# skokec/DAU-ConvNet

Hardware: AMD Instinct MI355X
Metric: DAU fwd+bwd GSamples/s (N*H*W/s) (higher is better)
Workload: dtype f32

## Files before the change

### dau-convnet_amd/csrc/k_dense_split.hip

```cpp
#include <algorithm>
#include <cstdint>
#include <cstdlib>
#include <type_traits>

#include "dau_tiled.hpp"

#ifndef DAU_SPLIT_R
#define DAU_SPLIT_R 3
#endif
#ifndef DAU_SPLIT_NS
#define DAU_SPLIT_NS s3
#endif

namespace dau {
namespace DAU_SPLIT_NS {

typedef _Float16 f16x8 __attribute__((ext_vector_type(8)));
typedef __attribute__((ext_vector_type(16))) float f32x16;
typedef __attribute__((ext_vector_type(4))) float f32x4;
typedef __attribute__((ext_vector_type(4))) unsigned u32x4;
typedef __attribute__((address_space(3))) void* lds_ptr_t;
typedef __attribute__((address_space(1))) const void* glb_ptr_t;

namespace {

constexpr int kDR = DAU_SPLIT_R;
constexpr int kDK = 2 * kDR + 1;
constexpr int kDSpan = kDK - 1;
constexpr int kDTaps = kDK * kDK;
constexpr int kDRows = 8;
constexpr int kDFB = 128;
constexpr int kAhead = 2;
#ifndef DAU_SPLIT_FLUSH_TAPS
#define DAU_SPLIT_FLUSH_TAPS 0
#endif
constexpr int kFlushTaps = DAU_SPLIT_FLUSH_TAPS > 0 ? DAU_SPLIT_FLUSH_TAPS : kDK;
#ifndef DAU_SPLIT_FLUSH_ROWS
#define DAU_SPLIT_FLUSH_ROWS 4
#endif
constexpr int kFlushRows = DAU_SPLIT_FLUSH_ROWS;
#if !defined(DAU_SPLIT_K32)
#if !defined(DAU_SPLIT_MFMA32) && DAU_SPLIT_R == 3
#define DAU_SPLIT_K32 1
#else
#define DAU_SPLIT_K32 0
#endif
#endif
constexpr bool kK32 = DAU_SPLIT_K32 != 0;

inline size_t round_up(size_t v, size_t a) { return (v + a - 1) / a * a; }

struct SplitScales {
    unsigned max_w_bits;
    float sw, inv_sw;
    float pad[5];
};
__host__ __device__ __forceinline__ const float* scales_sx(const SplitScales* sc) { return reinterpret_cast<const float*>(sc + 1); }
__host__ __device__ __forceinline__ const float* scales_inv_sx(const SplitScales* sc, int N) { return reinterpret_cast<const float*>(sc + 1) + N; }
constexpr int kPartials = 1024;
inline int absmax_groups_per_image(int N, long per) {
    const long fit = std::max(1, kPartials / N), want = (per / 4 + 255) / 256 + 1;
    return (int)std::min(fit, want);
}
inline size_t scales_bytes(int N) { return sizeof(SplitScales) + (size_t)2 * N * sizeof(float); }

constexpr int kMaxSub = 4;
struct SplitGeom {
    int sub;
    int nsub_a, nb_a, nsub_b, nb_b;
    int nrb8, nrb4;
    int tall;
    int Hs, Ws, nchunk, CoutP;
    size_t hdr_bytes, xs_bytes, ws_bytes;
};

SplitGeom split_geometry(const DenseConfig& c) {
    SplitGeom g{};
    g.sub = (c.W + 7) / 8;
    const int nblocks = (g.sub + kMaxSub - 1) / kMaxSub, base = g.sub / nblocks, rem = g.sub % nblocks;
    if (rem) { g.nsub_a = base + 1; g.nb_a = rem; g.nsub_b = base; g.nb_b = nblocks - rem; }
    else { g.nsub_a = base; g.nb_a = nblocks; g.nsub_b = 0; g.nb_b = 0; }
    const int left = c.H % kDRows;
    const long wgs = (long)c.N * ((c.H + kDRows - 1) / kDRows) * nblocks * ((c.Cout + kDFB - 1) / kDFB);
    const int rows4 = DAU_TUNE_INT("DAU_SPLIT_ROWS4", 1);
    g.nrb4 = (left >= 1 && left <= 4 && rows4 != 0 && (wgs >= 1024 || rows4 == 2)) ? 1 : 0;
    g.nrb8 = c.H / kDRows + (left && !g.nrb4 ? 1 : 0);
    g.Hs = g.nrb8 * kDRows + g.nrb4 * 4 + kDSpan;
    {
        const int t4 = (c.W + 3) / 4;
        const long rows8 = (long)g.nrb8 * kDRows;
        const long flat = (long)(g.nrb4 ? rows8 + 4 : (c.H + 3) / 4 * 4) * g.sub * 8;
        const long tall = rows8 * t4 * 4 + (g.nrb4 ? 4L * g.sub * 8 : 0);
        const int want = DAU_TUNE_INT("DAU_SPLIT_TALL", 1);
        g.tall = (want != 0 && g.nrb8 > 0 && (t4 == 5 || t4 == 7) && (tall * 20 <= flat * 19 || want == 2)) ? t4 : 0;
    }
    g.Ws = g.sub * 8 + kDSpan;
    g.nchunk = (c.Cin + 15) / 16;
    g.CoutP = (int)round_up(c.Cout, kDFB);
    g.hdr_bytes = round_up(scales_bytes(c.N) + (size_t)2 * (kPartials + c.N) * sizeof(unsigned), 256);
    g.xs_bytes = round_up((size_t)c.N * g.nchunk * 4 * g.Hs * g.Ws * 16 + 4096, 256);
    g.ws_bytes = round_up(((size_t)g.nchunk * kDTaps + 8) * 2 * g.CoutP * 32, 256);
    return g;
}

constexpr int lds_pitch(int nsub) {
    int p = nsub * 8 + kDSpan;
    while (p % 16 != 8) ++p;
    return p;
}
constexpr int lds_pitch_narrow(int ntiles) {
    int p = ntiles * 4 + kDSpan;
    while (p % 16 != 4 && p % 16 != 12) ++p;
    return p;
}

}

__device__ __forceinline__ unsigned finite_bits(unsigned b) { return b < 0x7f800000u ? b : 0u; }

__device__ __forceinline__ long absmax_head(const void* p, long per, int elem_bytes, int vec_bytes) {
    const uintptr_t a = reinterpret_cast<uintptr_t>(p);
    if (a % elem_bytes) return per;
    const long head = (long)((vec_bytes - a % vec_bytes) % vec_bytes) / elem_bytes;
    return head < per ? head : per;
}

__global__ void __launch_bounds__(256) split_absmax_kernel(const float* __restrict__ in, long per, int gpi, int act, const UnitRef* __restrict__ table,
                                                           long units, unsigned* __restrict__ partial, int cap, const Guard guard) {
    if (!guard_pass(guard)) return;
    unsigned mx = 0, mw = 0;
    const int n = blockIdx.x / gpi, j = blockIdx.x - n * gpi;
    const long stride = (long)gpi * blockDim.x, t0 = j * (long)blockDim.x + threadIdx.x;
    if (act == kActF16) {
        auto wide = [](unsigned h) { return finite_bits(__float_as_uint(f16_bits_to_float(h)) & 0x7fffffffu); };
        const unsigned short* e = reinterpret_cast<const unsigned short*>(in) + n * per;
        const long head = absmax_head(e, per, 2, 8), n4 = (per - head) / 4;
        const uint2* p = reinterpret_cast<const uint2*>(e + head);
        for (long i = t0; i < n4; i += stride) {
            const uint2 v = p[i];
            mx = max(mx, max(max(wide(v.x & 0xffffu), wide(v.x >> 16)), max(wide(v.y & 0xffffu), wide(v.y >> 16))));
        }
        for (long i = t0; i < per - n4 * 4; i += stride) mx = max(mx, wide(e[i < head ? i : i + n4 * 4]));
    } else if (act == kActBF16) {
        const unsigned short* e = reinterpret_cast<const unsigned short*>(in) + n * per;
        const long head = absmax_head(e, per, 2, 8), n4 = (per - head) / 4;
        const uint2* p = reinterpret_cast<const uint2*>(e + head);
        for (long i = t0; i < n4; i += stride) {
            const uint2 v = p[i];
            mx = max(mx, max(max(finite_bits((v.x << 16) & 0x7fffffffu), finite_bits(v.x & 0x7fff0000u)),
                             max(finite_bits((v.y << 16) & 0x7fffffffu), finite_bits(v.y & 0x7fff0000u))));
        }
        for (long i = t0; i < per - n4 * 4; i += stride) mx = max(mx, finite_bits(((unsigned)e[i < head ? i : i + n4 * 4] << 16) & 0x7fffffffu));
    } else {
        const float* e = in + n * per;
        const long head = absmax_head(e, per, 4, 16), n4 = (per - head) / 4;
        const uint4* p = reinterpret_cast<const uint4*>(e + head);
        for (long i = t0; i < n4; i += stride) {
            const uint4 v = p[i];
            mx = max(mx, max(max(finite_bits(v.x & 0x7fffffffu), finite_bits(v.y & 0x7fffffffu)),
                             max(finite_bits(v.z & 0x7fffffffu), finite_bits(v.w & 0x7fffffffu))));
        }
        for (long i = t0; i < per - n4 * 4; i += stride) mx = max(mx, finite_bits(__float_as_uint(e[i < head ? i : i + n4 * 4]) & 0x7fffffffu));
    }
    for (long u = blockIdx.x * (long)blockDim.x + threadIdx.x; u < units; u += (long)gridDim.x * blockDim.x) {
        const UnitRef r = table[u];
        mw = max(mw, finite_bits(__float_as_uint(fabsf(r.w00) + fabsf(r.w01) + fabsf(r.w10) + fabsf(r.w11))));
    }
    __shared__ unsigned sx[4], sw[4];
    for (int m = 32; m >= 1; m >>= 1) { mx = max(mx, (unsigned)__shfl_xor((int)mx, m)); mw = max(mw, (unsigned)__shfl_xor((int)mw, m)); }
    if ((threadIdx.x & 63) == 0) { sx[threadIdx.x >> 6] = mx; sw[threadIdx.x >> 6] = mw; }
    __syncthreads();
    if (threadIdx.x == 0) {
        partial[blockIdx.x] = max(max(sx[0], sx[1]), max(sx[2], sx[3]));
        partial[cap + blockIdx.x] = max(max(sw[0], sw[1]), max(sw[2], sw[3]));
    }
}

__device__ __forceinline__ float limb_scale(float m) {
    if (!(m > 0.0f) || !(m < INFINITY)) return 1.0f;
    int e = ilogbf(m);
    e = 13 - e;
    e = e > 100 ? 100 : (e < -100 ? -100 : e);
    return ldexpf(1.0f, e);
}

__global__ void __launch_bounds__(256) split_scales_kernel(const unsigned* __restrict__ partial, int N, int gpi, int cap, int G,
                                                           SplitScales* __restrict__ out, const Guard guard) {
    if (!guard_pass(guard)) return;
    const int n = blockIdx.x;
    const unsigned* src = n < N ? partial + (long)n * gpi : partial + cap;
    const int cnt = n < N ? gpi : N * gpi;
    unsigned m = 0;
    for (int i = threadIdx.x; i < cnt; i += 256) m = max(m, src[i]);
    __shared__ unsigned sm[4];
    for (int k = 32; k >= 1; k >>= 1) m = max(m, (unsigned)__shfl_xor((int)m, k));
    if ((threadIdx.x & 63) == 0) sm[threadIdx.x >> 6] = m;
    __syncthreads();
    if (threadIdx.x == 0) {
        m = max(max(sm[0], sm[1]), max(sm[2], sm[3]));
        float* sx = reinterpret_cast<float*>(out + 1);
        if (n < N) {
            const float s = limb_scale(__uint_as_float(m));
            sx[n] = s; sx[N + n] = 1.0f / s;
        } else {
            const float s = limb_scale(__uint_as_float(m) * (float)G);
            out->max_w_bits = m; out->sw = s; out->inv_sw = 1.0f / s;
        }
    }
}

constexpr int kScT = 64;
__global__ void __launch_bounds__(kScT) split_densify_kernel(const UnitRef* __restrict__ table, int Cin, int G, int Cout, int CoutP, int nchunk,
                                                             const SplitScales* __restrict__ sc, _Float16* __restrict__ wsd, const Guard guard) {
    __shared__ float acc[kDTaps * kScT];
    if (!guard_pass(guard)) return;
    constexpr int FPB = kScT / 16;
    const int tid = threadIdx.x, sl = tid & 15;
    const int fq = blockIdx.x % (CoutP / FPB), chunk = blockIdx.x / (CoutP / FPB);
    const int f = fq * FPB + (tid >> 4), c = chunk * 16 + sl;
#pragma unroll 7
    for (int tap = 0; tap < kDTaps; ++tap) acc[tap * kScT + tid] = 0.0f;
    if (c < Cin && f < Cout) {
        for (int g = 0; g < G; ++g) {
            const UnitRef u = table[((long)c * G + g) * Cout + f];
            const int ty = u.oy + kDR, tx = u.ox + kDR;
            const bool y0 = ty >= 0 && ty < kDK, y1 = ty + 1 >= 0 && ty + 1 < kDK, x0 = tx >= 0 && tx < kDK, x1 = tx + 1 >= 0 && tx + 1 < kDK;
            if (y0 && x0) acc[(ty * kDK + tx) * kScT + tid] += u.w00;
            if (y0 && x1) acc[(ty * kDK + tx + 1) * kScT + tid] += u.w01;
            if (y1 && x0) acc[((ty + 1) * kDK + tx) * kScT + tid] += u.w10;
            if (y1 && x1) acc[((ty + 1) * kDK + tx + 1) * kScT + tid] += u.w11;
        }
    }
    const float sw = sc->sw;
    _Float16* dst = wsd + ((long)chunk * kDTaps * 2 * CoutP + f) * 16 + sl;
    const long limb = (long)CoutP * 16, tapstride = 2 * limb;
#pragma unroll 7
    for (int tap = 0; tap < kDTaps; ++tap) {
        const float v = acc[tap * kScT + tid] * sw;
        const _Float16 hi = (_Float16)v;
        dst[tap * tapstride] = hi;
        dst[tap * tapstride + limb] = (_Float16)(v - (float)hi);
    }
}

constexpr int kSP = 80;
struct SplitStageArgs {
    const float* in;
    const float* taps;
    const SplitScales* sc;
    _Float16* xs;
    int N, C, H, W, mirrored;
    int Hs, Ws, nchunk;
    int RB, nbands, nsegs;
    int vec;
    Guard guard;
};

__device__ __forceinline__ int fast_div(int i, int d, float inv) {
    int q = (int)(((float)i + 0.5f) * inv);
    const int r = i - q * d;
    q += (r >= d) - (r < 0);
    return q;
}

template <int K, int NCH>
__device__ __forceinline__ void split_stage_rows(float* rawl, const float* px, int col, int ch0, int wave, int nw, int lh, int ncols) {
    constexpr int kr = (K - 1) / 2;
    if (col >= ncols) return;
    float gx[K];
#pragma unroll
    for (int j = 0; j < K; ++j) gx[j] = px[j];
    for (int r = wave; r < lh; r += nw) {
        float* row = rawl + (r * 8 + ch0) * kSP + 8 + col;
        float acc[NCH];
#pragma unroll
        for (int ch = 0; ch < NCH; ++ch) {
            acc[ch] = 0.0f;
#pragma unroll
            for (int i = 0; i < K; ++i) acc[ch] = fmaf(row[ch * kSP + i - kr], gx[i], acc[ch]);
        }
#pragma unroll
        for (int ch = 0; ch < NCH; ++ch) row[ch * kSP] = acc[ch];
    }
}

template <int K, int NCH>
__device__ __forceinline__ void split_stage_walk(const float* rawl, const float* py, float sx, int col, int ch0, int ya, int yb,
                                                 int y0, int x0, int x1, int Ws, u32x4* xhi, u32x4* xlo) {
    constexpr int kr = (K - 1) / 2;
    const int x = x0 + col;
    if (x >= x1) return;
    float gy[K];
#pragma unroll
    for (int j = 0; j < K; ++j) gy[j] = py[j];
    float ring[K][NCH];
    const int nin = yb - ya + 2 * kr;
    char* dhi = reinterpret_cast<char*>(xhi + (long)kDR * Ws + kDR + x) + ch0 * 2;
    char* dlo = reinterpret_cast<char*>(xlo + (long)kDR * Ws + kDR + x) + ch0 * 2;
    for (int s0 = 0; s0 < nin; s0 += K) {
#pragma unroll
        for (int j = 0; j < K; ++j) {
            const int s = s0 + j;
            if (s < nin) {
                const float* row = rawl + ((ya - y0 + s) * 8 + ch0) * kSP + 8 + col;
#pragma unroll
                for (int ch = 0; ch < NCH; ++ch) ring[j][ch] = row[ch * kSP];
                if (s >= K - 1) {
                    typedef _Float16 f16xn __attribute__((ext_vector_type(NCH)));
                    f16xn oh, ol;
#pragma unroll
                    for (int ch = 0; ch < NCH; ++ch) {
                        float acc = 0.0f;
#pragma unroll
                        for (int i = 0; i < K; ++i) acc = fmaf(ring[(j + 1 + i) % K][ch], gy[i], acc);
                        acc *= sx;
                        const _Float16 hi = (_Float16)acc;
                        oh[ch] = hi;
                        ol[ch] = (_Float16)(acc - (float)hi);
                    }
                    const long o = (long)(ya + s - (K - 1)) * Ws * 16;
                    *reinterpret_cast<f16xn*>(dhi + o) = oh;
                    *reinterpret_cast<f16xn*>(dlo + o) = ol;
                }
            }
        }
    }
}

#ifndef DAU_SPLIT_STAGE_THREADS
#define DAU_SPLIT_STAGE_THREADS 512
#endif
constexpr int kStageThreads = DAU_SPLIT_STAGE_THREADS;
template <int KN, int A>
__global__ void __launch_bounds__(kStageThreads) split_stage_kernel(const SplitStageArgs a) {
    constexpr int K = KN & (kNhwcArg - 1);
    constexpr bool NHWC = (KN & kNhwcArg) != 0;
    extern __shared__ __attribute__((aligned(16))) float rawl[];
    if (!guard_pass(a.guard)) return;
    constexpr int kr = (K - 1) / 2;
    constexpr int PPR = kSP / 4;
    const int lane = threadIdx.x & 63, wave = threadIdx.x >> 6, nw = blockDim.x >> 6;
    int t = blockIdx.x;
    const int seg = t % a.nsegs; t /= a.nsegs;
    const int band = t % a.nbands; t /= a.nbands;
    const int grp = t % (2 * a.nchunk);
    const int n = t / (2 * a.nchunk);
    const int y0 = band * a.RB, y1 = y0 + a.RB < a.H ? y0 + a.RB : a.H;
    const int x0 = seg * 64, x1 = x0 + 64 < a.W ? x0 + 64 : a.W;
    const int lh = y1 - y0 + 2 * kr;
    const long plane = (long)a.H * a.W;
    if constexpr (NHWC) {
        constexpr int CPP = A == kActF32 ? 4 : 8, PARTS = 8 / CPP;
        const int pieces = lh * kSP * PARTS;
        constexpr int UB = (13 * 256 + kStageThreads - 1) / kStageThreads;
        for (int i0 = threadIdx.x; i0 < pieces; i0 += kStageThreads * UB) {
            float v[UB][CPP];
#pragma unroll
            for (int u = 0; u < UB; ++u) {
                const int i = i0 + u * kStageThreads, part = i % PARTS, rj = i / PARTS, r = rj / kSP, j = rj - r * kSP;
                const int c = grp * 8 + part * CPP, y = y0 - kr + r, x = x0 - 8 + j;
                const bool pix = y >= 0 && y < a.H && x >= 0 && x < a.W && i < pieces;
                if (a.vec) {
                    const bool ok = pix && c < a.C;
                    const long idx = ok ? nhwc_index(n, c, y, x, a.C, a.H, a.W) : 0;
                    if constexpr (A == kActF32) {
                        const float4 w = *reinterpret_cast<const float4*>(a.in + idx);
                        v[u][0] = mask_act(w.x, ok); v[u][1] = mask_act(w.y, ok); v[u][2] = mask_act(w.z, ok); v[u][3] = mask_act(w.w, ok);
                    } else {
                        const uint4 w = *reinterpret_cast<const uint4*>(reinterpret_cast<const unsigned short*>(a.in) + idx);
                        const unsigned q[4] = {w.x, w.y, w.z, w.w};
#pragma unroll
                        for (int k = 0; k < 4; ++k) {
                            if constexpr (A == kActF16) {
                                v[u][2 * k] = mask_act(f16_bits_to_float(q[k] & 0xffffu), ok);
                                v[u][2 * k + 1] = mask_act(f16_bits_to_float(q[k] >> 16), ok);
                            } else {
                                const unsigned m = ok ? 0xffffffffu : 0u;
                                v[u][2 * k] = __uint_as_float((q[k] << 16) & m);
                                v[u][2 * k + 1] = __uint_as_float(q[k] & 0xffff0000u & m);
                            }
                        }
                    }
                } else {
#pragma unroll
                    for (int k = 0; k < CPP; ++k) {
                        const bool ok = pix && c + k < a.C;
                        v[u][k] = mask_act(load_act_t<A>(a.in, ok ? nhwc_index(n, c + k, y, x, a.C, a.H, a.W) : 0), ok);
                    }
                }
            }
#pragma unroll
            for (int u = 0; u < UB; ++u) {
                const int i = i0 + u * kStageThreads, part = i % PARTS, rj = i / PARTS, r = rj / kSP, j = rj - r * kSP;
                if (i < pieces) {
#pragma unroll
                    for (int k = 0; k < CPP; ++k) rawl[(r * 8 + part * CPP + k) * kSP + j] = v[u][k];
                }
            }
        }
    } else
    {
        const int pieces = lh * 8 * PPR;
        constexpr int UB = (13 * 256 + kStageThreads - 1) / kStageThreads;
        for (int i0 = threadIdx.x; i0 < pieces; i0 += kStageThreads * UB) {
            float4 v[UB];
#pragma unroll
            for (int u = 0; u < UB; ++u) {
                const int i = i0 + u * kStageThreads, rc = i / PPR, q = i - rc * PPR, r = rc >> 3, ch = rc & 7;
                const int c = grp * 8 + ch, y = y0 - kr + r, xs = x0 - 8 + 4 * q;
                const bool row_in = c < a.C && y >= 0 && y < a.H && i < pieces;
                const long base = ((long)n * a.C + (c < a.C ? c : 0)) * plane;
                if (a.vec) {
                    const bool ok = row_in && xs >= 0 && xs + 4 <= a.W;
                    const long idx = base + (ok ? (long)y * a.W + xs : 0);
                    if constexpr (A == kActF16) {
                        const uint2 w = *reinterpret_cast<const uint2*>(reinterpret_cast<const unsigned short*>(a.in) + idx);
                        v[u] = make_float4(mask_act(f16_bits_to_float(w.x & 0xffffu), ok), mask_act(f16_bits_to_float(w.x >> 16), ok),
                                           mask_act(f16_bits_to_float(w.y & 0xffffu), ok), mask_act(f16_bits_to_float(w.y >> 16), ok));
                    } else if constexpr (A == kActBF16) {
                        const uint2 w = *reinterpret_cast<const uint2*>(reinterpret_cast<const unsigned short*>(a.in) + idx);
                        const unsigned m = ok ? 0xffffffffu : 0u;
                        v[u] = make_float4(__uint_as_float((w.x << 16) & m), __uint_as_float(w.x & 0xffff0000u & m),
                                           __uint_as_float((w.y << 16) & m), __uint_as_float(w.y & 0xffff0000u & m));
                    } else {
                        const float4 w = *reinterpret_cast<const float4*>(a.in + idx);
                        v[u] = make_float4(mask_act(w.x, ok), mask_act(w.y, ok), mask_act(w.z, ok), mask_act(w.w, ok));
                    }
                } else {
                    float e[4];
#pragma unroll
                    for (int k = 0; k < 4; ++k) {
                        const bool ok = row_in && xs + k >= 0 && xs + k < a.W;
                        e[k] = mask_act(load_act_t<A>(a.in, base + (ok ? (long)y * a.W + xs + k : 0)), ok);
                    }
                    v[u] = make_float4(e[0], e[1], e[2], e[3]);
                }
            }
#pragma unroll
            for (int u = 0; u < UB; ++u) {
                const int i = i0 + u * kStageThreads;
                if (i < pieces) *reinterpret_cast<float4*>(rawl + (long)i * 4) = v[u];
            }
        }
    }
    const int chunk = grp >> 1, half = grp & 1;
    const long splane = (long)a.Hs * a.Ws;
    u32x4* xhi = reinterpret_cast<u32x4*>(a.xs) + ((((long)n * a.nchunk + chunk) * 2 + 0) * 2 + half) * splane;
    u32x4* xlo = xhi + 2 * splane;
    {
        const int rs0 = band == 0 ? 0 : y0 + kDR, rs1 = band == a.nbands - 1 ? a.Hs : y1 + kDR;
        const int cs0 = seg == 0 ? 0 : x0 + kDR, cs1 = seg == a.nsegs - 1 ? a.Ws : x1 + kDR;
        const int cw = cs1 - cs0, cnt = (rs1 - rs0) * cw;
        const float inv = 1.0f / (float)cw;
        const u32x4 z = {0u, 0u, 0u, 0u};
        for (int i = threadIdx.x; i < cnt; i += blockDim.x) {
            const int rr = fast_div(i, cw, inv), r = rs0 + rr, cc = cs0 + i - rr * cw;
            if (r >= y0 + kDR && r < y1 + kDR && cc >= x0 + kDR && cc < x1 + kDR) continue;
            xhi[(long)r * a.Ws + cc] = z;
            xlo[(long)r * a.Ws + cc] = z;
        }
    }
    __syncthreads();
    const float* px = a.taps + (a.mirrored ? kTapGXR : kTapGX) * kTapPitch;
    const float* py = a.taps + (a.mirrored ? kTapGYR : kTapGY) * kTapPitch;
    if (x1 - x0 <= 32) split_stage_rows<K, 4>(rawl, px, lane & 31, (lane >> 5) * 4, wave, nw, lh, x1 - x0);
    else split_stage_rows<K, 8>(rawl, px, lane, 0, wave, nw, lh, x1 - x0);
    __syncthreads();
    const int SR = (y1 - y0 + nw - 1) / nw;
    const int ya = y0 + wave * SR, yb = ya + SR < y1 ? ya + SR : y1;
    if (ya >= yb) return;
    const float sx = scales_sx(a.sc)[n];
    if (x1 - x0 <= 32) split_stage_walk<K, 4>(rawl, py, sx, lane & 31, (lane >> 5) * 4, ya, yb, y0, x0, x1, a.Ws, xhi, xlo);
    else split_stage_walk<K, 8>(rawl, py, sx, lane, 0, ya, yb, y0, x0, x1, a.Ws, xhi, xlo);
}

struct SplitArgs {
    const _Float16* xs;
    const _Float16* wsd;
    const SplitScales* sc;
    float* out;
    const float* partial;
    int N, Cout, CoutP, H, W, Hs, Ws, nchunk, ncb, nrb, out_act;
    int col0;
    int row0;
    Guard guard;
};
struct SplitArgsEpi : SplitArgs {
    const float* bias;
    int relu;
    const float* residual;
    int res_vec;
};

constexpr int kNhwcVecOut = 0x100;
template <int NSUBN, int RG = 2, bool TT = false, bool H16 = false, bool ADD = false>
__global__ void __launch_bounds__(512) split_gather_kernel(const typename std::conditional<(NSUBN & kEpiArg) != 0, SplitArgsEpi, SplitArgs>::type a) {
    constexpr int NSUB = NSUBN & (kNhwcArg - 1);
    constexpr bool NHWC = (NSUBN & kNhwcArg) != 0;
    constexpr bool EPI = (NSUBN & kEpiArg) != 0;
    static_assert(!TT || RG == 2, "tall tiles: blocks of eight rows");
    constexpr int TW = TT ? 4 : 8;
    constexpr int P = TT ? lds_pitch_narrow(NSUB) : lds_pitch(NSUB);
    constexpr int kRowsWG = 4 * RG;
    constexpr int NT0 = (RG == 2 && !TT) ? NSUB : (NSUB + 1) / 2;
    constexpr int NT1 = TT ? NSUB / 2 : NT0;
    constexpr int WR = kRowsWG + kDSpan;
    constexpr int PLANE = kK32 ? (WR * P + 15) / 16 * 16 : WR * P;
    constexpr int HALF = PLANE * 16;
    constexpr int BUFU = 4 * PLANE;
    constexpr int NPIECE = (BUFU + 63) / 64;
    constexpr int BUF1 = NPIECE * 1024;
    constexpr int BUF = kK32 ? 2 * BUF1 : BUF1;
    constexpr int PPW = (NPIECE + 7) / 8;
    extern __shared__ __attribute__((aligned(16))) char smem[];
    if (!guard_pass(a.guard)) return;
    const int lane = threadIdx.x & 63;
    const int wave = __builtin_amdgcn_readfirstlane(threadIdx.x >> 6);
    const int fw = wave & 3, pw = wave >> 2;
    const int prow = (RG == 2 && !TT) ? 4 * pw : 0, ptile = (RG == 2 && !TT) ? 0 : pw * NT0;
    int t;
#ifdef DAU_SPLIT_NO_XCD_MAP
    t = blockIdx.x;
#else
    {
        const int nblk = gridDim.x, xcd = blockIdx.x % 8, idx = blockIdx.x / 8;
        const int per = nblk / 8, rem = nblk % 8;
        t = (xcd < rem ? xcd * (per + 1) : rem * (per + 1) + (xcd - rem) * per) + idx;
    }
#endif
    const int fb = t % (a.CoutP / kDFB); t /= (a.CoutP / kDFB);
    const int cb = t % a.ncb; t /= a.ncb;
    const int rb = t % a.nrb;
    const int n = t / a.nrb;
    const int h = lane >> 5, nn = lane & 31;

    const long xs_plane = (long)a.Hs * a.Ws;
    const int colb = a.col0 + cb * NSUB * TW;
    const int rowb = a.row0 + rb * kRowsWG;
    const u32x4* xsrc = reinterpret_cast<const u32x4*>(a.xs) + ((long)n * a.nchunk * 4) * xs_plane + (long)rowb * a.Ws + colb;
    int goff[PPW];
#pragma unroll
    for (int i = 0; i < PPW; ++i) {
        int piece = wave + 8 * i;
        piece = piece < NPIECE ? piece : NPIECE - 1;
        int L = piece * 64 + lane;
        L = L < BUFU ? L : BUFU - 1;
        const int ph = L / PLANE;
        int rem = L - ph * PLANE;
        rem = rem < WR * P ? rem : WR * P - 1;
        const int r = rem / P, c = rem - r * P;
        goff[i] = (int)(ph * xs_plane + (long)r * a.Ws + c);
    }
    auto issue = [&](int chunk, int buf) {
        const u32x4* src = xsrc + (long)chunk * 4 * xs_plane;
#pragma unroll
        for (int i = 0; i < PPW; ++i) {
            int piece = wave + 8 * i;
            piece = piece < NPIECE ? piece : NPIECE - 1;
            __builtin_amdgcn_global_load_lds((glb_ptr_t)(src + goff[i]), (lds_ptr_t)(smem + buf * BUF + piece * 1024), 16, 0, 0);
        }
        if constexpr (kK32) {
            if (chunk + 1 < a.nchunk) {
#pragma unroll
                for (int i = 0; i < PPW; ++i) {
                    int piece = wave + 8 * i;
                    piece = piece < NPIECE ? piece : NPIECE - 1;
                    __builtin_amdgcn_global_load_lds((glb_ptr_t)(src + 4 * xs_plane + goff[i]), (lds_ptr_t)(smem + buf * BUF + BUF1 + piece * 1024), 16, 0, 0);
                }
            }
        }
    };

    const int prr = TT ? nn >> 2 : nn >> 3, pcc = TT ? nn & 3 : nn & 7;
    float* const out_ptr = a.out;
    const float* const part_ptr = a.partial;
    const bool out_bf16 = NHWC ? (a.out_act & 0xff) != 0 : a.out_act != 0;
    const bool vec_out = NHWC && (a.out_act & kNhwcVecOut) != 0;
    const int out_c = a.Cout, out_h = a.H, out_w = a.W;
    const float* bias_ptr = nullptr;
    const float* res_ptr = nullptr;
    bool relu = false, vec_res = false;
    if constexpr (EPI) { bias_ptr = a.bias; relu = a.relu != 0; }
    auto read_residual = [&](float tie) __attribute__((always_inline)) {
        if constexpr (EPI) {
            unsigned long kargs = (unsigned long)__builtin_amdgcn_kernarg_segment_ptr();
            asm volatile("" : "+s"(kargs) : "v"(tie));
            const auto* late = reinterpret_cast<const __attribute__((address_space(4))) SplitArgsEpi*>(kargs);
            res_ptr = late->residual;
            vec_res = NHWC && late->res_vec != 0;
        }
    };
    auto finished = [&](float v, int f, float r) __attribute__((always_inline)) {
        const int fc = f < out_c ? f : out_c - 1;
        return epilogue_value(v, bias_ptr ? bias_ptr[fc] : 0.0f, bias_ptr != nullptr, relu, r, res_ptr != nullptr);
    };
    auto residual_at = [&](long o) __attribute__((always_inline)) {
        if constexpr (H16) return load_act_t<kActF16>(res_ptr, o);
        else return out_bf16 ? load_act_t<kActBF16>(res_ptr, o) : res_ptr[o];
    };
    auto joined = [&](float s, float inv_w, float inv_x, float part) __attribute__((always_inline)) {
        float v = s * inv_w * inv_x + part;
        if constexpr (H16) asm("" : "+v"(v));
        return v;
    };
    auto store4 = [&](int y, int x, bool tile, int f0, const float (&s)[4], float inv_w, float inv_x) __attribute__((always_inline)) {
        const long plane = (long)out_h * out_w;
        if (!(y < out_h && x < out_w && tile)) return;
        if constexpr (NHWC) {
            const long pix = ((long)n * out_h + y) * out_w + x;
            float v[4];
            float r[4] = {0.0f, 0.0f, 0.0f, 0.0f};
            if constexpr (EPI) {
                if (res_ptr) {
                    const long o = pix * out_c + f0;
                    if (vec_res) {
                        if (f0 < out_c) {
                            if constexpr (H16) {
                                typedef _Float16 f16x4 __attribute__((ext_vector_type(4)));
                                const f16x4 q = *reinterpret_cast<const f16x4*>(reinterpret_cast<const unsigned short*>(res_ptr) + o);
#pragma unroll
                                for (int k = 0; k < 4; ++k) r[k] = (float)q[k];
                            } else if (out_bf16) {
                                const uint2 q = *reinterpret_cast<const uint2*>(reinterpret_cast<const unsigned short*>(res_ptr) + o);
                                r[0] = __uint_as_float(q.x << 16); r[1] = __uint_as_float(q.x & 0xffff0000u);
                                r[2] = __uint_as_float(q.y << 16); r[3] = __uint_as_float(q.y & 0xffff0000u);
                            } else {
// ... 230 lines not shown
            xb[0][0] = read(0, 0); xb[0][1] = read(0, 1); xb[1][0] = read(1, 0); xb[1][1] = read(1, 1);
            __builtin_amdgcn_sched_group_barrier(0x100, 4, 0);
#pragma unroll
            for (int u = 0; u < U; ++u) {
                const int tx = u / NG, p = u % NG;
                if (u + 2 < U) { xb[(u + 2) % 3][0] = read(u + 2, 0); xb[(u + 2) % 3][1] = read(u + 2, 1); }
                const f16x8 xh = xb[u % 3][0], xl = xb[u % 3][1];
                const f16x8 h0 = ah[tx][0], h1 = ah[tx][1], l0 = al[tx][0], l1 = al[tx][1];
                const bool fresh = kFlushRows == 1 && tx % kFlushTaps == 0;
                acc[p][0] = __builtin_amdgcn_mfma_f32_16x16x32_f16(h0, xh, fresh ? zero : acc[p][0], 0, 0, 0);
                acc[p][1] = __builtin_amdgcn_mfma_f32_16x16x32_f16(h1, xh, fresh ? zero : acc[p][1], 0, 0, 0);
                if (p == 0) {
                    if (tx + kAhead < kDK) {
#pragma unroll
                        for (int m = 0; m < 2; ++m) { ah[tx + kAhead][m] = load_a(wcur, (tx + kAhead) * wtap, m); al[tx + kAhead][m] = load_a(wcur, (tx + kAhead) * wtap + wlo, m); }
                    }
                    if (tx == kDK - 3 || tx == kDK - 2) {
                        const int i = tx - (kDK - 3);
#pragma unroll
                        for (int m = 0; m < 2; ++m) { an[i][m] = load_a(wnxt, i * wtap, m); bn[i][m] = load_a(wnxt, i * wtap + wlo, m); }
                    }
                }
                acc[p][0] = __builtin_amdgcn_mfma_f32_16x16x32_f16(l0, xh, acc[p][0], 0, 0, 0);
                acc[p][1] = __builtin_amdgcn_mfma_f32_16x16x32_f16(l1, xh, acc[p][1], 0, 0, 0);
                acc[p][0] = __builtin_amdgcn_mfma_f32_16x16x32_f16(h0, xl, acc[p][0], 0, 0, 0);
                acc[p][1] = __builtin_amdgcn_mfma_f32_16x16x32_f16(h1, xl, acc[p][1], 0, 0, 0);
                if (u + 2 < U) __builtin_amdgcn_sched_group_barrier(0x100, 2, 0);
                __builtin_amdgcn_sched_group_barrier(0x008, 2, 0);
                if (p == 0 && tx + kAhead < kDK && tx == kDK - 3) __builtin_amdgcn_sched_group_barrier(0x020, 8, 0);
                else if (p == 0 && (tx + kAhead < kDK || tx == kDK - 2)) __builtin_amdgcn_sched_group_barrier(0x020, 4, 0);
                __builtin_amdgcn_sched_group_barrier(0x008, 4, 0);
                if ((tx + 1) % kFlushTaps == 0 && tx + 1 < kDK) { sum[p][0] += acc[p][0]; sum[p][1] += acc[p][1]; }
            }
#pragma unroll
            for (int m = 0; m < 2; ++m) { ah[0][m] = an[0][m]; al[0][m] = bn[0][m]; ah[1][m] = an[1][m]; al[1][m] = bn[1][m]; }
            if constexpr (kFlushRows == 1) {
#pragma unroll
                for (int p = 0; p < NG; ++p) { sum[p][0] += acc[p][0]; sum[p][1] += acc[p][1]; }
            } else {
                if (++rows_chained == kFlushRows) {
                    rows_chained = 0;
#pragma unroll
                    for (int p = 0; p < NG; ++p) { sum[p][0] += acc[p][0]; sum[p][1] += acc[p][1]; acc[p][0] = zero; acc[p][1] = zero; }
                }
            }
        }
        if (more) {
            asm volatile("s_waitcnt vmcnt(0)" ::: "memory");
            __syncthreads();
        }
    }
    if constexpr (kFlushRows > 1) {
#pragma unroll
        for (int p = 0; p < NG; ++p) { sum[p][0] += acc[p][0]; sum[p][1] += acc[p][1]; }
    }
    const float inv_w = a.sc->inv_sw, inv_x = scales_inv_sx(a.sc, a.N)[n];
    read_residual(sum[0][0][0]);
#pragma unroll
    for (int p = 0; p < NG; ++p) {
        const int y = rowb + prow + (p & 1) * GR + qr, x = colb + TW * (ptile + (p >> 1)) + qc;
#pragma unroll
        for (int m = 0; m < 2; ++m) {
            const float s4[4] = {sum[p][m][0], sum[p][m][1], sum[p][m][2], sum[p][m][3]};
            store4(y, x, ptile + (p >> 1) < NSUB, fb * kDFB + fw * 32 + 16 * m + 4 * g, s4, inv_w, inv_x);
        }
    }
    };
    auto run = [&](auto ntc) __attribute__((always_inline)) {
        if constexpr (kK32) body32(ntc);
        else body(ntc);
    };
    if constexpr (TT) {
        if (pw == 0) run(std::integral_constant<int, NT0>{});
        else run(std::integral_constant<int, NT1>{});
    } else {
        run(std::integral_constant<int, NT0>{});
    }
}

namespace {

template <int NSUB, int RG, bool TT>
constexpr size_t split_lds_bytes() {
    constexpr int plane = (4 * RG + kDSpan) * (TT ? lds_pitch_narrow(NSUB) : lds_pitch(NSUB));
    return (kK32 ? 4 : 2) * (size_t)((4 * (kK32 ? (plane + 15) / 16 * 16 : plane) + 63) / 64) * 1024;
}

template <int NSUB, int RG, bool TT = false>
void launch_split(hipStream_t st, const SplitArgsEpi* a, int grid, bool h16, bool add, bool nhwc, bool epi) {
    constexpr int NH = NSUB | kNhwcArg;
    constexpr int EP = NSUB | kEpiArg, EH = NH | kEpiArg;
    constexpr size_t lds = split_lds_bytes<NSUB, RG, TT>();
    if (epi) {
        auto kern = h16 ? split_gather_kernel<EP, RG, TT, true> : split_gather_kernel<EP, RG, TT, false>;
        if (nhwc) kern = h16 ? split_gather_kernel<EH, RG, TT, true> : split_gather_kernel<EH, RG, TT, false>;
#if DAU_SPLIT_R == 3
        if (add) kern = h16 ? split_gather_kernel<EP, RG, TT, true, true> : split_gather_kernel<EP, RG, TT, false, true>;
        if (add && nhwc) kern = h16 ? split_gather_kernel<EH, RG, TT, true, true> : split_gather_kernel<EH, RG, TT, false, true>;
#endif
        if (!a) { (void)hipFuncSetAttribute(reinterpret_cast<const void*>(kern), hipFuncAttributeMaxDynamicSharedMemorySize, 160 * 1024); return; }
        hipLaunchKernelGGL(kern, dim3(grid), dim3(512), lds, st, *a);
        return;
    }
    auto kern = h16 ? split_gather_kernel<NSUB, RG, TT, true> : split_gather_kernel<NSUB, RG, TT, false>;
    if (nhwc) kern = h16 ? split_gather_kernel<NH, RG, TT, true> : split_gather_kernel<NH, RG, TT, false>;
#if DAU_SPLIT_R == 3
    if (add) kern = h16 ? split_gather_kernel<NSUB, RG, TT, true, true> : split_gather_kernel<NSUB, RG, TT, false, true>;
    if (add && nhwc) kern = h16 ? split_gather_kernel<NH, RG, TT, true, true> : split_gather_kernel<NH, RG, TT, false, true>;
#endif
    if (!a) { (void)hipFuncSetAttribute(reinterpret_cast<const void*>(kern), hipFuncAttributeMaxDynamicSharedMemorySize, 160 * 1024); return; }
    hipLaunchKernelGGL(kern, dim3(grid), dim3(512), lds, st, static_cast<const SplitArgs&>(*a));
}

void dispatch_split(int nsub, int rg, bool h16, hipStream_t st, const SplitArgsEpi* a, int grid, bool tall, bool add, bool nhwc, bool epi) {
    if (tall) {
        if (nsub == 5) launch_split<5, 2, true>(st, a, grid, h16, add, nhwc, epi);
        else launch_split<7, 2, true>(st, a, grid, h16, add, nhwc, epi);
        return;
    }
    if (rg == 1) {
        switch (nsub) {
            case 1: launch_split<1, 1>(st, a, grid, h16, add, nhwc, epi); break;
            case 2: launch_split<2, 1>(st, a, grid, h16, add, nhwc, epi); break;
            case 3: launch_split<3, 1>(st, a, grid, h16, add, nhwc, epi); break;
            default: launch_split<4, 1>(st, a, grid, h16, add, nhwc, epi); break;
        }
        return;
    }
    switch (nsub) {
        case 1: launch_split<1, 2>(st, a, grid, h16, add, nhwc, epi); break;
        case 2: launch_split<2, 2>(st, a, grid, h16, add, nhwc, epi); break;
        case 3: launch_split<3, 2>(st, a, grid, h16, add, nhwc, epi); break;
        default: launch_split<4, 2>(st, a, grid, h16, add, nhwc, epi); break;
    }
}

const void* stage_for(int blur_k, int act, bool nhwc = false) {
#define DAU_SPLIT_STAGE(K) case K: if (nhwc) return act == kActF16 ? reinterpret_cast<const void*>(split_stage_kernel<K | kNhwcArg, kActF16>) : \
                                          act == kActBF16 ? reinterpret_cast<const void*>(split_stage_kernel<K | kNhwcArg, kActBF16>) : \
                                                            reinterpret_cast<const void*>(split_stage_kernel<K | kNhwcArg, kActF32>); \
                                   return act == kActF16 ? reinterpret_cast<const void*>(split_stage_kernel<K, kActF16>) : \
                                          act == kActBF16 ? reinterpret_cast<const void*>(split_stage_kernel<K, kActBF16>) : \
                                                            reinterpret_cast<const void*>(split_stage_kernel<K, kActF32>)
    switch (blur_k) {
        DAU_SPLIT_STAGE(3);
        DAU_SPLIT_STAGE(5);
        DAU_SPLIT_STAGE(7);
        DAU_SPLIT_STAGE(9);
        DAU_SPLIT_STAGE(11);
        default: return nullptr;
    }
#undef DAU_SPLIT_STAGE
}
void stage_plan(const DenseConfig& c, int* RB, int* nbands, size_t* lds) {
    const int kr = (c.blur_k - 1) / 2;
    int rows = 52 * 1024 / (8 * kSP * 4) - 2 * kr;
    const int rb = DAU_TUNE_INT("DAU_SPLIT_STAGE_RB", 0);
    if (rb > 0) rows = rb;
    rows = rows < 4 ? 4 : rows;
    const int nb = (c.H + rows - 1) / rows;
    *nbands = nb; *RB = (c.H + nb - 1) / nb;
    *lds = (size_t)(*RB + 2 * kr) * 8 * kSP * 4;
}

}

bool split_gather_configure(int N, int Cin, int Cout, int G, int H, int W, int R, int blur_k, int act, DenseConfig* cfg) {
    if (R != kDR || !stage_for(blur_k, act)) return false;
    DenseConfig c{};
    c.N = N; c.Cin = Cin; c.Cout = Cout; c.G = G; c.H = H; c.W = W; c.R = R; c.blur_k = blur_k; c.act = act;
    const SplitGeom g = split_geometry(c);
    c.nsub = g.nsub_a;
    c.ftiles = 1;
    if ((size_t)g.nchunk * 4 * g.Hs * g.Ws > (size_t)1 << 30) return false;
    *cfg = c;
    return true;
}

size_t split_gather_workspace_bytes(const DenseConfig& c) {
    const SplitGeom g = split_geometry(c);
    return g.hdr_bytes + g.xs_bytes + g.ws_bytes;
}

void split_gather_init(const DenseConfig& c) {
    const SplitGeom g = split_geometry(c);
    const bool h16 = c.act == kActF16;
    for (int rg = 1; rg <= 2; ++rg) {
        if (!(rg == 2 ? g.nrb8 : g.nrb4)) continue;
        for (int v = 0; v < (kDR == 3 ? 4 : 2); ++v) {
            const bool add = (v & 2) != 0, epi = (v & 1) != 0;
            if (rg == 2 && g.tall) { dispatch_split(g.tall, 2, h16, nullptr, nullptr, 0, true, add, c.nhwc != 0, epi); continue; }
            dispatch_split(g.nsub_a, rg, h16, nullptr, nullptr, 0, false, add, c.nhwc != 0, epi);
            if (g.nb_b) dispatch_split(g.nsub_b, rg, h16, nullptr, nullptr, 0, false, add, c.nhwc != 0, epi);
        }
    }
    (void)hipFuncSetAttribute(stage_for(c.blur_k, c.act, c.nhwc != 0), hipFuncAttributeMaxDynamicSharedMemorySize, 160 * 1024);
}

void split_gather_prepare(hipStream_t st, const DenseConfig& c, const float* in, const float* filters, bool mirrored,
                          const UnitRef* table, void* workspace, const Guard& guard) {
    const SplitGeom g = split_geometry(c);
    char* ws = static_cast<char*>(workspace);
    SplitScales* sc = reinterpret_cast<SplitScales*>(ws);
    unsigned* partial = reinterpret_cast<unsigned*>(ws + scales_bytes(c.N));
    _Float16* xs = reinterpret_cast<_Float16*>(ws + g.hdr_bytes);
    _Float16* wsd = reinterpret_cast<_Float16*>(ws + g.hdr_bytes + g.xs_bytes);
    const long per = (long)c.Cin * c.H * c.W, units = (long)c.Cin * c.G * c.Cout;
    const int gpi = absmax_groups_per_image(c.N, per), cap = kPartials + c.N;
    hipLaunchKernelGGL(split_absmax_kernel, dim3(c.N * gpi), dim3(256), 0, st, in, per, gpi, c.act, table, units, partial, cap, guard);
    hipLaunchKernelGGL(split_scales_kernel, dim3(c.N + 1), dim3(256), 0, st, partial, c.N, gpi, cap, c.G, sc, guard);
    hipLaunchKernelGGL(split_densify_kernel, dim3(g.nchunk * (g.CoutP / (kScT / 16))), dim3(kScT), 0, st, table, c.Cin, c.G, c.Cout, g.CoutP,
                       g.nchunk, sc, wsd, guard);
    SplitStageArgs s{};
    s.in = in; s.taps = filters + kTaps1dOffset; s.sc = sc; s.xs = xs;
    s.N = c.N; s.C = c.Cin; s.H = c.H; s.W = c.W; s.mirrored = mirrored ? 1 : 0;
    s.Hs = g.Hs; s.Ws = g.Ws; s.nchunk = g.nchunk; s.guard = guard;
    size_t lds;
    stage_plan(c, &s.RB, &s.nbands, &lds);
    s.nsegs = (c.W + 63) / 64;
    s.vec = c.W % 4 == 0 && reinterpret_cast<uintptr_t>(in) % 16 == 0;
    if (c.nhwc) s.vec = c.Cin % (c.act == kActF32 ? 4 : 8) == 0 && reinterpret_cast<uintptr_t>(in) % 16 == 0;
    void* args[] = {&s};
    (void)hipLaunchKernel(stage_for(c.blur_k, c.act, c.nhwc != 0), dim3(c.N * 2 * g.nchunk * s.nbands * s.nsegs), dim3(kStageThreads), args, lds, st);
}

namespace {
void run_split(hipStream_t st, const DenseConfig& c, float* out, const float* partial, void* workspace, const Guard& guard,
               const Epilogue& epilogue) {
    const SplitGeom g = split_geometry(c);
    const bool add = partial != nullptr;
    const bool h16 = c.act == kActF16;
    char* ws = static_cast<char*>(workspace);
    SplitArgsEpi a{};
    a.sc = reinterpret_cast<const SplitScales*>(ws);
    a.xs = reinterpret_cast<const _Float16*>(ws + g.hdr_bytes);
    a.wsd = reinterpret_cast<const _Float16*>(ws + g.hdr_bytes + g.xs_bytes);
    a.out = out; a.partial = partial;
    a.N = c.N; a.Cout = c.Cout; a.CoutP = g.CoutP; a.H = c.H; a.W = c.W; a.Hs = g.Hs; a.Ws = g.Ws; a.nchunk = g.nchunk;
    a.out_act = c.act; a.guard = guard;
    a.bias = epilogue.bias; a.relu = epilogue.relu ? 1 : 0; a.residual = epilogue.residual;
    const bool epi = epilogue.on();
    const bool nhwc = c.nhwc != 0;
    if (nhwc && c.Cout % 4 == 0 && reinterpret_cast<uintptr_t>(out) % (c.act == kActF32 ? 16 : 8) == 0) a.out_act |= kNhwcVecOut;
    a.res_vec = epilogue.residual && nhwc && c.Cout % 4 == 0 && reinterpret_cast<uintptr_t>(epilogue.residual) % (c.act == kActF32 ? 16 : 8) == 0;
    for (int rg = 2; rg >= 1; --rg) {
        a.nrb = rg == 2 ? g.nrb8 : g.nrb4;
        if (!a.nrb) continue;
        a.row0 = rg == 2 ? 0 : g.nrb8 * kDRows;
        if (rg == 2 && g.tall) {
            a.ncb = 1; a.col0 = 0;
            dispatch_split(g.tall, 2, h16, st, &a, c.N * a.nrb * (g.CoutP / kDFB), true, add, nhwc, epi);
            continue;
        }
        a.ncb = g.nb_a; a.col0 = 0;
        dispatch_split(g.nsub_a, rg, h16, st, &a, c.N * a.nrb * g.nb_a * (g.CoutP / kDFB), false, add, nhwc, epi);
        if (g.nb_b) {
            a.ncb = g.nb_b; a.col0 = g.nb_a * g.nsub_a * 8;
            dispatch_split(g.nsub_b, rg, h16, st, &a, c.N * a.nrb * g.nb_b * (g.CoutP / kDFB), false, add, nhwc, epi);
        }
    }
}
}

void split_gather_run(hipStream_t st, const DenseConfig& c, float* out, void* workspace, const Guard& guard, const Epilogue& epi) {
    run_split(st, c, out, nullptr, workspace, guard, epi);
}

#if DAU_SPLIT_R == 3
void split_gather_run_add(hipStream_t st, const DenseConfig& c, float* out, const float* partial, void* workspace, const Guard& guard,
                          const Epilogue& epi) {
    run_split(st, c, out, partial, workspace, guard, epi);
}

SplitStaged split_gather_staged(const DenseConfig& c, const void* workspace) {
    const SplitGeom g = split_geometry(c);
    const char* ws = static_cast<const char*>(workspace);
    SplitStaged s{};
    s.sx = scales_sx(reinterpret_cast<const SplitScales*>(ws));
    s.xs = reinterpret_cast<const _Float16*>(ws + g.hdr_bytes);
    s.Hs = g.Hs; s.Ws = g.Ws; s.nchunk = g.nchunk;
    return s;
}
#endif

}
}
```

Before: 0.01835.

## Add single-wave streaming row-walk kernel for split staging blur

Adds a new staging kernel that runs one wave per block, stream-loads input rows with a prefetch depth, does the horizontal blur from a double-buffered LDS row and keeps the vertical blur in a register ring, then writes the hi/lo fp16 split. It replaces the block-wide LDS-band staging path for NCHW inputs, so block barriers and large LDS tiles go away in favour of wave-level syncs and register pipelining. Band and segment counts are chosen to give roughly 2048 waves. Risks are register pressure from the unrolled ring and prefetch buffers, and redundant halo row loads at band edges.

```diff
diff --git a/dau-convnet_amd/csrc/k_dense_split.hip b/dau-convnet_amd/csrc/k_dense_split.hip
--- a/dau-convnet_amd/csrc/k_dense_split.hip
+++ b/dau-convnet_amd/csrc/k_dense_split.hip
@@ -2,6 +2,7 @@
 #include <cstdint>
 #include <cstdlib>
 #include <type_traits>
+#include <utility>
 
 #include "dau_tiled.hpp"
 
@@ -252,6 +253,7 @@
     int N, C, H, W, mirrored;
     int Hs, Ws, nchunk;
     int RB, nbands, nsegs;
+    int TW;
     int vec;
     Guard guard;
 };
@@ -472,6 +474,154 @@
     const float sx = scales_sx(a.sc)[n];
     if (x1 - x0 <= 32) split_stage_walk<K, 4>(rawl, py, sx, lane & 31, (lane >> 5) * 4, ya, yb, y0, x0, x1, a.Ws, xhi, xlo);
     else split_stage_walk<K, 8>(rawl, py, sx, lane, 0, ya, yb, y0, x0, x1, a.Ws, xhi, xlo);
+}
+
+typedef float f32x2 __attribute__((ext_vector_type(2)));
+__device__ __forceinline__ void stage_wave_sync() {
+    __builtin_amdgcn_fence(__ATOMIC_RELEASE, "wavefront");
+    __builtin_amdgcn_wave_barrier();
+    __builtin_amdgcn_fence(__ATOMIC_ACQUIRE, "wavefront");
+}
+template <int N, class F>
+__device__ __forceinline__ void stage_unroll(F&& f) {
+    [&]<int... I>(std::integer_sequence<int, I...>) { (f(std::integral_constant<int, I>{}), ...); }(std::make_integer_sequence<int, N>{});
+}
+#ifndef DAU_SPLIT_WALK_AHEAD
+#define DAU_SPLIT_WALK_AHEAD 2
+#endif
+constexpr int stage_walk_buf(int K) { return (8 * (64 + K - 1) + 63) / 64 * 64; }
+
+template <int K, int A, int NCH>
+__device__ __forceinline__ void split_stage_walk_tile(const SplitStageArgs& a, float* lds, int n, int grp, int cs0, int cs1, int b0, int b1) {
+    typedef typename RawAct<A>::type Raw;
+    typedef _Float16 f16xn __attribute__((ext_vector_type(NCH)));
+    constexpr int kr = (K - 1) / 2, CW = (NCH == 8 ? 64 : 32) + K - 1, kBuf = stage_walk_buf(K);
+    constexpr int CWL = CW < 64 ? CW : 64, XT = CW - CWL, NX = (8 * XT + 63) / 64, NL = 8 + NX;
+    constexpr int kAhead = K > 3 ? DAU_SPLIT_WALK_AHEAD : 2;
+    static_assert(8 * CW <= kBuf, "the eight channels' rows lie inside the row buffer");
+    const int lane = threadIdx.x, col = NCH == 8 ? lane : lane & 31, ch0 = NCH == 8 ? 0 : (lane >> 5) * 4;
+    const int H = a.H, W = a.W;
+    const long plane = (long)H * W;
+    const float* px = a.taps + (a.mirrored ? kTapGXR : kTapGX) * kTapPitch;
+    const float* py = a.taps + (a.mirrored ? kTapGYR : kTapGY) * kTapPitch;
+    f32x2 gx[K], gy[K];
+#pragma unroll
+    for (int j = 0; j < K; ++j) { gx[j] = f32x2{px[j], px[j]}; gy[j] = f32x2{py[j], py[j]}; }
+    const int xm = cs0 - kDR - kr + lane;
+    const bool okm = lane < CWL && xm >= 0 && xm < W;
+    const unsigned offm = (unsigned)(xm < 0 ? 0 : xm < W ? xm : W - 1);
+    unsigned offx[NX > 0 ? NX : 1], posx[NX > 0 ? NX : 1], okx = 0u;
+#pragma unroll
+    for (int e = 0; e < NX; ++e) {
+        const int tt = e * 64 + lane, tc = tt < 8 * XT ? tt : 0;
+        const int ch = XT > 0 ? tc / (XT > 0 ? XT : 1) : 0, cl = 64 + tc - ch * XT;
+        const bool chan = grp * 8 + ch < a.C;
+        const int xx = cs0 - kDR - kr + cl;
+        okx |= (tt < 8 * XT ? 1u : 0u) << (2 * e) | (tt < 8 * XT && chan && xx >= 0 && xx < W ? 2u : 0u) << (2 * e);
+        offx[e] = (unsigned)((chan ? ch : 0) * plane) + (unsigned)(xx < 0 ? 0 : xx < W ? xx : W - 1);
+        posx[e] = (unsigned)((ch >> 1) * 2 * CW + cl * 2 + (ch & 1));
+    }
+    const long gbase = ((long)n * a.C + (grp * 8 < a.C ? grp * 8 : 0)) * plane;
+    const float sx = scales_sx(a.sc)[n];
+    const int steps = (b1 - b0 + K - 1 + K - 1) / K * K;
+    Raw rv[K][NL];
+    f32x2 ring[K][NCH / 2];
+#pragma unroll
+    for (int i = 0; i < K; ++i)
+#pragma unroll
+        for (int cp = 0; cp < NCH / 2; ++cp) ring[i][cp] = f32x2{0.0f, 0.0f};
+    auto load_row = [&](int u, Raw* dst) {
+        const int r = b0 - kDR - kr + u, rc = r < 0 ? 0 : r < H ? r : H - 1;
+        const long rowbase = gbase + (long)rc * W;
+#pragma unroll
+        for (int l = 0; l < 8; ++l) dst[l] = load_raw<A>(a.in, rowbase + (grp * 8 + l < a.C ? l : 0) * plane + (long)offm);
+#pragma unroll
+        for (int e = 0; e < NX; ++e) dst[8 + e] = load_raw<A>(a.in, rowbase + (long)offx[e]);
+    };
+#pragma unroll
+    for (int d = 0; d < kAhead; ++d) load_row(d, rv[d]);
+    const int chunk = grp >> 1, half = grp & 1;
+    const long splane = (long)a.Hs * a.Ws;
+    u32x4* const xhi = reinterpret_cast<u32x4*>(a.xs) + ((((long)n * a.nchunk + chunk) * 2 + 0) * 2 + half) * splane;
+    u32x4* const xlo = xhi + 2 * splane;
+    const int cs = cs0 + col, x = cs - kDR;
+    const bool col_in = x >= 0 && x < W, col_st = cs < cs1;
+    auto step = [&](auto pc, int u) {
+        constexpr int P = decltype(pc)::value;
+        load_row(u + kAhead, rv[(P + kAhead) % K]);
+        const int r = b0 - kDR - kr + u;
+        const bool row_in = r >= 0 && r < H;
+        float* buf = lds + (u & 1) * kBuf;
+        if (CWL == 64 || lane < CWL) {
+#pragma unroll
+            for (int l = 0; l < 8; ++l)
+                buf[(l >> 1) * 2 * CW + lane * 2 + (l & 1)] = mask_act(act_of(rv[P][l]), okm && row_in && grp * 8 + l < a.C);
+        }
+#pragma unroll
+        for (int e = 0; e < NX; ++e)
+            if ((okx >> (2 * e)) & 1u) buf[posx[e]] = mask_act(act_of(rv[P][8 + e]), ((okx >> (2 * e)) & 2u) && row_in);
+        stage_wave_sync();
+        f32x2 h[NCH / 2];
+#pragma unroll
+        for (int cp = 0; cp < NCH / 2; ++cp) h[cp] = f32x2{0.0f, 0.0f};
+        const f32x2* row = reinterpret_cast<const f32x2*>(buf) + (ch0 / 2) * CW + col;
+#pragma unroll
+        for (int c0 = 0; c0 < NCH / 2; c0 += 2) {
+            stage_unroll<K>([&](auto ic) {
+                constexpr int I = decltype(ic)::value;
+#pragma unroll
+                for (int cp = c0; cp < c0 + 2; ++cp) h[cp] = __builtin_elementwise_fma(row[cp * CW + I], gx[I], h[cp]);
+            });
+            __builtin_amdgcn_sched_barrier(0);
+        }
+#pragma unroll
+        for (int cp = 0; cp < NCH / 2; ++cp) ring[P][cp] = h[cp];
+        const int rs = b0 + u - (K - 1), y = rs - kDR;
+        f32x2 o[NCH / 2];
+#pragma unroll
+        for (int cp = 0; cp < NCH / 2; ++cp) o[cp] = f32x2{0.0f, 0.0f};
+        stage_unroll<K>([&](auto jc) {
+            constexpr int J = decltype(jc)::value, sl = (P + 1 + J) % K;
+#pragma unroll
+            for (int cp = 0; cp < NCH / 2; ++cp) o[cp] = __builtin_elementwise_fma(ring[sl][cp], gy[J], o[cp]);
+        });
+        const bool in = col_in && y >= 0 && y < H;
+        f16xn oh, ol;
+#pragma unroll
+        for (int ch = 0; ch < NCH; ++ch) {
+            float acc = o[ch / 2][ch & 1];
+            acc *= sx;
+            const _Float16 hi = (_Float16)acc;
+            oh[ch] = in ? hi : (_Float16)0.0f;
+            ol[ch] = in ? (_Float16)(acc - (float)hi) : (_Float16)0.0f;
+        }
+        if (col_st && rs >= b0 && rs < b1) {
+            const long o16 = ((long)rs * a.Ws + cs) * 16 + ch0 * 2;
+            *reinterpret_cast<f16xn*>(reinterpret_cast<char*>(xhi) + o16) = oh;
+            *reinterpret_cast<f16xn*>(reinterpret_cast<char*>(xlo) + o16) = ol;
+        }
+    };
+#pragma unroll 1
+    for (int u0 = 0; u0 < steps; u0 += K) {
+        stage_unroll<K>([&](auto pc) { step(pc, u0 + decltype(pc)::value); });
+    }
+}
+
+#ifndef DAU_SPLIT_WALK_WAVES
+#define DAU_SPLIT_WALK_WAVES 4
+#endif
+template <int K, int A>
+__global__ void __launch_bounds__(64) __attribute__((amdgpu_waves_per_eu(K <= 7 ? DAU_SPLIT_WALK_WAVES : 2))) split_stage_walk_kernel(const SplitStageArgs a) {
+    __shared__ __attribute__((aligned(16))) float lds[2 * stage_walk_buf(K)];
+    if (!guard_pass(a.guard)) return;
+    int t = blockIdx.x;
+    const int seg = t % a.nsegs; t /= a.nsegs;
+    const int band = t % a.nbands; t /= a.nbands;
+    const int grp = t % (2 * a.nchunk), n = t / (2 * a.nchunk);
+    const int cs0 = seg * a.TW, cs1 = cs0 + a.TW < a.Ws ? cs0 + a.TW : a.Ws;
+    const int b0 = band * a.RB, b1 = b0 + a.RB < a.Hs ? b0 + a.RB : a.Hs;
+    if (a.TW <= 32) split_stage_walk_tile<K, A, 4>(a, lds, n, grp, cs0, cs1, b0, b1);
+    else split_stage_walk_tile<K, A, 8>(a, lds, n, grp, cs0, cs1, b0, b1);
 }
 
 struct SplitArgs {
@@ -1008,6 +1158,35 @@
     }
 #undef DAU_SPLIT_STAGE
 }
+const void* stage_walk_for(int blur_k, int act) {
+#ifdef DAU_SPLIT_STAGE_REF
+    return nullptr;
+#else
+#define DAU_SPLIT_STAGE_WALK(K) case K: return act == kActF16 ? reinterpret_cast<const void*>(split_stage_walk_kernel<K, kActF16>) : \
+                                               act == kActBF16 ? reinterpret_cast<const void*>(split_stage_walk_kernel<K, kActBF16>) : \
+                                                                 reinterpret_cast<const void*>(split_stage_walk_kernel<K, kActF32>)
+    switch (blur_k) {
+        DAU_SPLIT_STAGE_WALK(3);
+        DAU_SPLIT_STAGE_WALK(5);
+        DAU_SPLIT_STAGE_WALK(7);
+        DAU_SPLIT_STAGE_WALK(9);
+        DAU_SPLIT_STAGE_WALK(11);
+        default: return nullptr;
+    }
+#undef DAU_SPLIT_STAGE_WALK
+#endif
+}
+void stage_walk_plan(const DenseConfig& c, const SplitGeom& g, SplitStageArgs* s) {
+    s->nsegs = (g.Ws + 63) / 64;
+    s->TW = (g.Ws + s->nsegs - 1) / s->nsegs;
+    s->nsegs = (g.Ws + s->TW - 1) / s->TW;
+    const long waves = (long)c.N * 2 * g.nchunk * s->nsegs;
+    long nb = (2048 + waves - 1) / waves;
+    nb = std::min<long>(nb, std::max(1, g.Hs / (2 * c.blur_k)));
+    const int rb = DAU_TUNE_INT("DAU_SPLIT_STAGE_WALK_RB", 0);
+    s->RB = rb > 0 ? rb : (int)((g.Hs + nb - 1) / nb);
+    s->nbands = (g.Hs + s->RB - 1) / s->RB;
+}
 void stage_plan(const DenseConfig& c, int* RB, int* nbands, size_t* lds) {
     const int kr = (c.blur_k - 1) / 2;
     int rows = 52 * 1024 / (8 * kSP * 4) - 2 * kr;
@@ -1071,6 +1250,12 @@
     s.in = in; s.taps = filters + kTaps1dOffset; s.sc = sc; s.xs = xs;
     s.N = c.N; s.C = c.Cin; s.H = c.H; s.W = c.W; s.mirrored = mirrored ? 1 : 0;
     s.Hs = g.Hs; s.Ws = g.Ws; s.nchunk = g.nchunk; s.guard = guard;
+    if (const void* walk = c.nhwc ? nullptr : stage_walk_for(c.blur_k, c.act)) {
+        stage_walk_plan(c, g, &s);
+        void* args[] = {&s};
+        (void)hipLaunchKernel(walk, dim3(c.N * 2 * g.nchunk * s.nbands * s.nsegs), dim3(64), args, 0, st);
+        return;
+    }
     size_t lds;
     stage_plan(c, &s.RB, &s.nbands, &lds);
     s.nsegs = (c.W + 63) / 64;
```

Result: faster. 0.01876, median of 6 (+2.2%).
